# dorukb/Advanced-CPU-Raytracing

Measured on AMD Instinct MI355X. Metric: Mrays/sec + achieved HBM GB/s fraction, 1920×1080 primary+shadow rays, higher is better.
Workload: dtype f32; 1 GPU; synthetic height field K=100352 tris, 1920x1080, 1 spp, 1 point light, default Blinn-Phong, primary+shadow rays; scene_K=100352, width=1920, height=1080, spp=1, rays_per_frame=4147193, camera_rays=2073600, frames_in_flight=16

## Files before the change

advanced-cpu-raytracing_amd/csrc/rtg_common.hpp:

```cpp
#pragma once
#include <hip/hip_runtime.h>
#include <stdint.h>

#include "rtg_device.hpp"

#ifndef RTG_MEGA_WAVES
#define RTG_MEGA_WAVES 2
#endif
#if RTG_MEGA_WAVES > 2 && !defined(RTG_MEGA_WAVES_EXPERIMENTAL)
#error "RTG_MEGA_WAVES > 2 is experimental (round-1 scratch fault, DESIGN.md §7): add -DRTG_MEGA_WAVES_EXPERIMENTAL=1"
#endif
#ifndef RTG_LEAN_WAVES
#define RTG_LEAN_WAVES 8
#endif
#ifndef RTG_SHADE_WAVES
#define RTG_SHADE_WAVES 3
#endif
#ifndef RTG_TREE_SHADE_WAVES
#define RTG_TREE_SHADE_WAVES 1
#endif
#ifndef RTG_BIGLEAF_LEAN
#define RTG_BIGLEAF_LEAN 0
#endif
#ifndef RTG_INST_WAVES
// ... 344 lines not shown
        hit = tt & (t > 0.0f) & (t < limit);
    }
    const bool unsure = !no & !tt;
    if (__builtin_expect(__ballot(unsure) != 0, 0)) {
        if (unsure) hit = tri_test_rec(R, r, limit, tout);
    }
    return hit;
}

DEV float tri_test_pk(const float4* R, const Ray& r, float limit, float& tout, float onf) {
    const float4 A = R[0], E1 = R[1], E2 = R[2];
    const float dx = r.d.x, dy = r.d.y, dz = r.d.z;
    const float detA = det3(E1.x, E2.x, dx, E1.y, E2.y, dy, E1.z, E2.z, dz);
    const float ad = fabsf(detA);
    const float rd = __builtin_amdgcn_rcpf(detA);
    const float sx = A.x - r.o.x, sy = A.y - r.o.y, sz = A.z - r.o.z;
    const float nb = det3(sx, E2.x, dx, sy, E2.y, dy, sz, E2.z, dz);
    const float ng = det3(E1.x, sx, dx, E1.y, sy, dy, E1.z, sz, dz);
    const float beta = nb * rd, gama = ng * rd, sum = gama + beta;
    const float sslack = fmaf(0x1p-19f, sum, 0x1p-22f);
    const float rng = __builtin_elementwise_minimum(ad - 0x1p-100f, 0x1p100f - ad);
    const float ttv = __builtin_elementwise_minimum(vmin3(beta - 1e-30f, gama - 1e-30f, (1.0f - sum) - sslack),
                                                    __builtin_elementwise_minimum(rng, onf));
    const float rjv = __builtin_elementwise_minimum(fmaxf(fmaxf(-1e-30f - beta, -1e-30f - gama), (sum - 1.0f) - sslack),
                                                    rng);
    float hv = -1.0f;
    if (__ballot(ttv > 0.0f)) {
        const float t = det3(E1.x, E2.x, sx, E1.y, E2.y, sy, E1.z, E2.z, sz) / detA;
        tout = t;
        hv = vmin3(ttv, t, limit - t);
    }
    const bool unsure = (onf > 0.0f) & !(ttv > 0.0f) & !(rjv > 0.0f) & (detA != 0.0f);
    if (__builtin_expect(__ballot(unsure) != 0, 0)) {
        if (unsure) hv = tri_test_rec(R, r, limit, tout) ? 1.0f : -1.0f;
    }
    return hv;
}

typedef int rtg_s16 __attribute__((ext_vector_type(16)));
typedef int rtg_s8 __attribute__((ext_vector_type(8)));
typedef int rtg_s4 __attribute__((ext_vector_type(4)));
DEV const void* uniform_ptr(const void* p) {
    const uint64_t v = (uint64_t)p;
    const uint32_t lo = __builtin_amdgcn_readfirstlane((uint32_t)v), hi = __builtin_amdgcn_readfirstlane((uint32_t)(v >> 32));
    return (const void*)(((uint64_t)hi << 32) | lo);
}
DEV void sload_wnode(const WNode* p, rtg_s16& a, rtg_s16& b) {
    asm volatile("s_load_dwordx16 %0, %2, 0x0\n\ts_load_dwordx16 %1, %2, 0x40\n\ts_waitcnt lgkmcnt(0)"
                 : "=&s"(a), "=&s"(b) : "s"(uniform_ptr(p)) : "memory");
}
DEV void sload_rec(const float4* p, rtg_s8& a, rtg_s4& b) {
    asm volatile("s_load_dwordx8 %0, %2, 0x0\n\ts_load_dwordx4 %1, %2, 0x20\n\ts_waitcnt lgkmcnt(0)"
                 : "=&s"(a), "=&s"(b) : "s"(uniform_ptr(p)) : "memory");
}
DEV void sload_node(const float4* p, rtg_s8& a) {
    asm volatile("s_load_dwordx8 %0, %1, 0x0\n\ts_waitcnt lgkmcnt(0)" : "=&s"(a) : "s"(uniform_ptr(p)) : "memory");
}
DEV float4 f4(int x, int y, int z, int w) {
    return make_float4(__int_as_float(x), __int_as_float(y), __int_as_float(z), __int_as_float(w));
}
DEV uint64_t hit_key(float t, int f) { return ((uint64_t)__float_as_uint(t) << 32) | (uint32_t)f; }

DEV uint64_t shfl64(uint64_t v, int src) {
    const uint32_t lo = (uint32_t)__shfl((int)(uint32_t)v, src);
    const uint32_t hi = (uint32_t)__shfl((int)(uint32_t)(v >> 32), src);
    return ((uint64_t)hi << 32) | lo;
}
DEV uint64_t wave_min_key(uint64_t key, uint64_t em) {
    if (em == ~0ull) {
        const int lane = threadIdx.x & 63;
        for (int m = 1; m < 64; m <<= 1) {
            const uint64_t other = shfl64(key, lane ^ m);
            if (other < key) key = other;
        }
        return key;
    }
    uint64_t acc = ~0ull;
    while (em) {
        const int l = __ffsll((long long)em) - 1;
        em &= em - 1;
        const uint64_t v = shfl64(key, l);
        if (v < acc) acc = v;
    }
    return acc;
}

#ifndef RTG_SEQ_SEL
#define RTG_SEQ_SEL 1
#endif
template <bool ANY, bool STATS, bool SEL = RTG_SEQ_SEL != 0>
DEV bool walk_bvh_seq(const DevScene& S, int i, const int end, const Ray& r, float& minT, int& hitFace, float limit,
                      Cnt<STATS>& c) {
    bool hit = false;
    const RayRcp q = ray_rcp(r);
    while (i < end) {
        const float4 a = S.nodes[2 * i];
        const float4 b = S.nodes[2 * i + 1];
        c.template node<ANY>();
        const int skip = __float_as_int(b.z);
        if (box_hit_fast<SEL>(a.x, a.y, a.z, a.w, b.x, b.y, r, q, minT)) {
            const int leaf = __float_as_int(b.w);
            if (leaf >= 0) {
                int first = leaf >> 8, cnt = leaf & 255;
                if (leaf == LEAF_EXT) {
                    const int2 e = S.node_ext[i];
                    first = e.x;
                    cnt = e.y;
                }
                for (int f = first; f < first + cnt; ++f) {
                    c.template tri<ANY>();
                    float t;
                    if (SEL ? tri_test_sel(S.tris + 3 * f, r, minT, t) : tri_test_fast(S, f, r, minT, t)) {
                        minT = t;
                        hitFace = f;
                        hit = true;
                        if (ANY && t < limit) return true;
                    }
                }
                i = skip;
            } else {
                i = i + 1;
            }
        } else {
            i = skip;
        }
    }
    return hit;
}


struct SlabRay {
    f3 o;
    float ix, iy, iz;
};
DEV SlabRay slab_ray(const Ray& r, const RayRcp& q) {
    SlabRay s;
    s.o = r.o;
    s.ix = q.ix; s.iy = q.iy; s.iz = q.iz;
    return s;
}
DEV bool slab_cons(float lx, float ly, float lz, float hx, float hy, float hz, const SlabRay& s, float minTc,
                   float& tnear) {
    const float tx1 = (lx - s.o.x) * s.ix, tx2 = (hx - s.o.x) * s.ix;
    const float ty1 = (ly - s.o.y) * s.iy, ty2 = (hy - s.o.y) * s.iy;
    const float tz1 = (lz - s.o.z) * s.iz, tz2 = (hz - s.o.z) * s.iz;
    const float tmin = fmaxf(fmaxf(fminf(tx1, tx2), fminf(ty1, ty2)), fminf(tz1, tz2));
    const float tmax = fminf(fminf(fmaxf(tx1, tx2), fmaxf(ty1, ty2)), fmaxf(tz1, tz2));
    tnear = tmin;
    return (tmax > -1e-30f) & (tmax >= fmaf(tmin, 1.0f - 0x1p-21f, -1e-30f)) & (tmin < minTc);
}

struct CoopEvent {
    float ox, oy, oz, dx, dy, dz, minT;
    int first, cnt, start;
    unsigned long long best;
};
DEV void wave_lds_sync() {
    __builtin_amdgcn_fence(__ATOMIC_RELEASE, "wavefront");
    __builtin_amdgcn_wave_barrier();
    __builtin_amdgcn_fence(__ATOMIC_ACQUIRE, "wavefront");
}
DEV uint64_t coop_leaf_tests(const DevScene& S, uint64_t coop, const Ray& r, float minT, int first, int cnt) {
    __shared__ CoopEvent table[4][64];
    CoopEvent* E = table[threadIdx.x >> 6];
    const uint64_t em = __ballot(1);
    const int lane = threadIdx.x & 63;
    const int nact = __popcll(em);
    const int rank = __popcll(em & ((1ull << lane) - 1ull));
    const int ne = __popcll(coop);
    const int slot = cnt > 0 ? __popcll(coop & ((1ull << lane) - 1ull)) : -1;
    if (slot >= 0) {
        CoopEvent& e = E[slot];
        e.ox = r.o.x; e.oy = r.o.y; e.oz = r.o.z;
        e.dx = r.d.x; e.dy = r.d.y; e.dz = r.d.z;
        e.minT = minT;
        e.first = first;
        e.cnt = cnt;
        e.best = ~0ull;
    }
    wave_lds_sync();
    int total = 0, start = 0;
    for (int k = 0; k < ne; ++k) {
        if (k == slot) start = total;
        total += E[k].cnt;
    }
    if (slot >= 0) E[slot].start = start;
    wave_lds_sync();
    for (int w = rank; w < total; w += nact) {
        int lo = 0, hi = ne - 1;
        while (lo < hi) {
            const int mid = (lo + hi + 1) >> 1;
            if (E[mid].start <= w) lo = mid;
            else hi = mid - 1;
        }
        const CoopEvent& e = E[lo];
        Ray lr;
        lr.o = mk(e.ox, e.oy, e.oz);
        lr.d = mk(e.dx, e.dy, e.dz);
        const int f = e.first + (w - e.start);
        float t;
        if (tri_test_fast(S, f, lr, e.minT, t)) atomicMin(&E[lo].best, (unsigned long long)hit_key(t, f));
    }
    wave_lds_sync();
    const uint64_t mine = slot >= 0 ? (uint64_t)E[slot].best : ~0ull;
    wave_lds_sync();
    return mine;
}

template <bool ANY, bool STATS, bool COOP>
DEV bool walk_bvh(const DevScene& S, int i, const int end, const Ray& r, float& minT, int& hitFace, float limit,
                  Cnt<STATS>& c) {
    if constexpr (!COOP) return walk_bvh_seq<ANY, STATS>(S, i, end, r, minT, hitFace, limit, c);
    if (!S.coop) return walk_bvh_seq<ANY, STATS, false>(S, i, end, r, minT, hitFace, limit, c);
    bool hit = false;
    const RayRcp q = ray_rcp(r);
    bool active = i < end;
    while (__ballot(active)) {
        int coopFirst = 0, coopCnt = 0;
        if (active) {
            const float4 a = S.nodes[2 * i];
            const float4 b = S.nodes[2 * i + 1];
            c.template node<ANY>();
            const int skip = __float_as_int(b.z);
            if (box_hit_fast(a.x, a.y, a.z, a.w, b.x, b.y, r, q, minT)) {
                const int leaf = __float_as_int(b.w);
                if (leaf >= 0) {
                    int first = leaf >> 8, cnt = leaf & 255;
                    if (leaf == LEAF_EXT) {
                        const int2 e = S.node_ext[i];
                        first = e.x;
                        cnt = e.y;
                    }
                    if (cnt > kCoopLeaf) {
                        coopFirst = first;
                        coopCnt = cnt;
                    } else {
                        for (int f = first; f < first + cnt; ++f) {
                            c.template tri<ANY>();
                            float t;
                            if (tri_test_fast(S, f, r, minT, t)) {
                                minT = t;
                                hitFace = f;
                                hit = true;
                                if (ANY && t < limit) {
                                    active = false;
                                    break;
                                }
                            }
                        }
                    }
                    i = skip;
                } else {
                    i = i + 1;
                }
            } else {
                i = skip;
            }
            if (i >= end) active = false;
        }
        const uint64_t coop = __ballot(coopCnt > 0);
        if (coop) {
            const uint64_t best = coop_leaf_tests(S, coop, r, minT, coopFirst, coopCnt);
            if (coopCnt > 0) {
                c.template tri_n<ANY>((uint32_t)coopCnt);
                if (best != ~0ull) {
                    minT = __uint_as_float((uint32_t)(best >> 32));
                    hitFace = (int)(uint32_t)best;
                    hit = true;
                    if (ANY && minT < limit) active = false;
                }
            }
        }
    }
    return hit;
}

DEV int wave_min_int(int v) {
    for (int m = 1; m < 64; m <<= 1) {
        const int o = __shfl_xor(v, m);
        v = o < v ? o : v;
    }
    return v;
}

constexpr int kDeferLeaf = 16;
template <int BYTES, typename T>
DEV const T* rec_at(const T* base, int i) {
    return (const T*)((const char*)base + (uint32_t)i * (uint32_t)BYTES);
}
#ifndef RTG_DEFER_LANES
#define RTG_DEFER_LANES 16
#endif
struct DeferCtx {
    float4* e;
    int* count;
    int cap;
    int ray;
    bool deferred;
};
DEV uint64_t obj_key(float t, int k, int f) {
    return ((uint64_t)__float_as_uint(t) << 32) | ((uint64_t)(uint32_t)k << 20) | (uint64_t)((uint32_t)f & 0xFFFFFu);
}

template <bool ANY, bool STATS, bool SC = false, bool DEFER = false>
DEV bool walk_bvh_packet(const DevScene& S, int begin, int end, const Ray& r, float& minT, int& hitFace,
                         float limit, Cnt<STATS>& c, DeferCtx* dc = nullptr, int k = 0) {
    begin = __builtin_amdgcn_readfirstlane(begin);
    end = __builtin_amdgcn_readfirstlane(end);
    const int face0 = hitFace;
    bool hit = false;
    const RayRcp q = ray_rcp(r);
    const SlabFma sf = slab_fma(r, q);
    const float slack0 = slab_slack0(sf, q.fast);
    const int kDone = 0x7FFFFFFF;
    int resume = begin;
    int i = begin;
    while (i < end) {
        bool act = resume <= i;
        if (ANY && !__ballot(act)) {
            const int all = __ballot(1) == ~0ull ? wave_min_int(resume) : [&] {
                int m = kDone;
                uint64_t em = __ballot(1);
                while (em) {
                    const int l = __ffsll((long long)em) - 1;
                    em &= em - 1;
                    const int v = __shfl(resume, l);
                    m = v < m ? v : m;
                }
                return m;
            }();
            i = __builtin_amdgcn_readfirstlane(all);
            continue;
        }
        i = __builtin_amdgcn_readfirstlane(i);
        const int ip1 = i + 1;
        float4 a, b;
        int ndr[8];
        if constexpr (SC) {
            rtg_s8 nd;
            sload_node(rec_at<32>(S.nodes, i), nd);
            a = f4(nd[0], nd[1], nd[2], nd[3]);
            b = f4(nd[4], nd[5], nd[6], nd[7]);
#pragma unroll
            for (int u = 0; u < 8; ++u) ndr[u] = nd[u];
        } else {
            a = S.nodes[2 * i];
            b = S.nodes[2 * i + 1];
        }
        const int skip = __float_as_int(b.z);
        const int leaf = __float_as_int(b.w);
        bool pass;
        if constexpr (SC) {
            if (act) c.template node<ANY>();
            pass = box_pass_pk(a.x, a.y, a.z, a.w, b.x, b.y, r, sf, minT, ip1 - resume, slack0);
            resume = max(resume, pass ? 0 : skip);
        } else {
            pass = false;
            if (act) {
                c.template node<ANY>();
                pass = box_hit_fast(a.x, a.y, a.z, a.w, b.x, b.y, r, q, minT);
                if (!pass) resume = skip;
            }
        }
        const int cur = i;
        int lf;
        {
            const uint64_t pm = __builtin_amdgcn_ballot_w64(pass);
            int nx;
            asm("s_cmp_lg_u64 %[pm], 0\n\t"
                "s_cselect_b32 %[lf], %[leaf], 0\n\t"
                "s_cmp_lt_i32 %[lf], 0\n\t"
                "s_cselect_b32 %[nx], %[ip1], %[skip]"
                : [lf] "=&s"(lf), [nx] "=&s"(nx)
                : [pm] "s"(pm), [leaf] "s"(leaf), [ip1] "s"(ip1), [skip] "s"(skip)
                : "scc");
            i = nx;
        }
        if (lf > 0) {
            {
                int first = leaf >> 8, cnt = leaf & 255;
                if (leaf == LEAF_EXT) {
                    const int2 e = S.node_ext[cur];
                    first = __builtin_amdgcn_readfirstlane(e.x);
                    cnt = __builtin_amdgcn_readfirstlane(e.y);
                }
                if constexpr (DEFER) {
                    const uint64_t m = __ballot(pass);
                    if (cnt > kDeferLeaf && __popcll(m) <= RTG_DEFER_LANES) {
                        const int lane = threadIdx.x & 63, lead = __ffsll((long long)m) - 1;
                        int base = 0;
                        if (lane == lead) base = atomicAdd(dc->count, __popcll(m));
                        base = __shfl(base, lead);
                        const int slot = base + __popcll(m & ((1ull << lane) - 1ull));
                        if (pass && slot < dc->cap) {
                            float4* q = dc->e + 3 * (size_t)slot;
                            q[0] = make_float4(r.o.x, r.o.y, r.o.z, minT);
                            q[1] = make_float4(r.d.x, r.d.y, r.d.z, __int_as_float(dc->ray));
                            q[2] = make_float4(__int_as_float(first), __int_as_float(cnt), __int_as_float(k), 0.f);
                            dc->deferred = true;
                            pass = false;
                        }
                    }
                }
                for (int f = first; f < first + cnt; ++f) {
                    if constexpr (SC) {
                        rtg_s8 ra;
                        rtg_s4 rb;
                        sload_rec(rec_at<48>(S.tris, f), ra, rb);
                        const float4 R[3] = {f4(ra[0], ra[1], ra[2], ra[3]), f4(ra[4], ra[5], ra[6], ra[7]),
                                             f4(rb[0], rb[1], rb[2], rb[3])};
                        if (pass) c.template tri<ANY>();
                        float t;
                        const bool ok = tri_test_pk(R, r, minT, t, pass ? 1.0f : -1.0f) > 0.0f;
                        minT = ok ? t : minT;
                        hitFace = ok ? f : hitFace;
                        if (ANY) {
                            const bool fin = ok & (t < limit);
                            pass &= !fin;
                            resume = fin ? kDone : resume;
                        }
                    } else if (pass) {
                        c.template tri<ANY>();
                        float t;
                        if (tri_test_fast(S, f, r, minT, t)) {
                            minT = t;
                            hitFace = f;
                            hit = true;
                            if (ANY && t < limit) {
                                pass = false;
                                resume = kDone;
                            }
                        }
                    }
                }
            }
        }
    }
    if constexpr (SC) return hit | (hitFace != face0);
    return hit;
}

#ifndef RTG_XFORM_LAUNDER
#define RTG_XFORM_LAUNDER 1
#endif
DEV bool sphere_t(const DevObject& ob, const Ray& lr, float minT, float& tout) {
    const f3 center = mk(ob.center[0], ob.center[1], ob.center[2]);
    const float radius = ob.center[3];
    f3 oc = sub(lr.o, center);
    float c = dot(oc, oc) - (radius * radius);
    float b = 2 * dot(lr.d, oc);
    float a = dot(lr.d, lr.d);
    float delta = b * b - (4 * a * c);
    if (delta < 0.0f) return false;
    delta = sqrtf(delta);
    a = (float)(2.0 * a);
    float t1 = (-b + delta) / a;
    float t2 = (-b - delta) / a;
    float t = t1 < t2 ? t1 : t2;
    if (t1 < t2) { t = (t1 > 0.0f) ? t1 : t2; }
    else if (t2 < t1) { t = (t2 > 0.0f) ? t2 : t1; }
    tout = t;
    return t < minT && t > 0.0f;
}

template <bool MOTION = true>
DEV Ray local_ray(const DevObject& ob, const Ray& r, float mbTime) {
    Ray lr;
    lr.o = xform(ob.inv, r.o, 1.0f);
    lr.d = xform(ob.inv, r.d, 0.0f);
    if (MOTION && (ob.flags & OBJF_MOTION_BLUR)) lr.o = add(lr.o, muls(ld3(ob.mbv), mbTime));
    return lr;
}
DEV Ray trav_ray(const DevObject& ob, const Ray& r0, float mbTime) {
    Ray r = r0;
#if RTG_XFORM_LAUNDER
    asm volatile("" : "+v"(r.o.x), "+v"(r.o.y), "+v"(r.o.z), "+v"(r.d.x), "+v"(r.d.y), "+v"(r.d.z));
#endif
    if (!(ob.flags & OBJF_IDENTITY)) return local_ray(ob, r, mbTime);
    Ray lr = ident_ray(r);
    if (ob.flags & OBJF_MOTION_BLUR) lr.o = add(lr.o, muls(ld3(ob.mbv), mbTime));
    return lr;
}

struct Hit {
    float t;
    int obj, face;
    f3 o;
};

template <bool ANY, bool STATS, int FEAT = FEAT_ALL, bool PK = false, bool DEFER = false>
DEV bool trace(const DevScene& S, Ray& r, float mbTime, float minT, float limit, Hit& h, Cnt<STATS>& c,
               DeferCtx* dc = nullptr) {
    h.t = minT;
    h.obj = -1;
    h.face = -1;
    const RayRcp rq = (FEAT & FEAT_INSTANCE) ? ray_rcp(r) : RayRcp{};
    int gskip = 0;
    for (int k = 0; k < S.num_objects; ++k) {
        const DevObject& ob = S.objects[k];
        if ((FEAT & FEAT_INSTANCE) && ob.group_end > k) {
            const float4 ga = S.group_box[2 * k], gb = S.group_box[2 * k + 1];
            if constexpr (PK) {
                if (k >= gskip && !box_hit_fast(ga.x, ga.y, ga.z, gb.x, gb.y, gb.z, r, rq, h.t)) gskip = ob.group_end;
                if (!__ballot(k >= gskip)) {
                    k = ob.group_end - 1;
                    continue;
                }
            } else if (!box_hit_fast(ga.x, ga.y, ga.z, gb.x, gb.y, gb.z, r, rq, h.t)) {
                k = ob.group_end - 1;
                continue;
            }
        }
        if (PK && k < gskip) continue;
        c.obj();
        if ((FEAT & FEAT_SPHERE) && ob.kind == OBJ_SPHERE) {
            c.sph();
            Ray lr = trav_ray(ob, r, mbTime);
            float t;
            if (sphere_t(ob, lr, h.t, t)) {
                h.t = t; h.obj = k; h.face = -1; h.o = r.o;
                if (ANY && t < limit) return true;
            }
            continue;
        }
        if (ANY && (ob.flags & OBJF_SHADOW_SKIP)) continue;
        if ((FEAT & FEAT_INSTANCE) && ob.kind == OBJ_INSTANCE) {
            Ray wr = r;
            if (ob.flags & OBJF_MOTION_BLUR) wr.o = add(wr.o, muls(ld3(ob.mbv), mbTime));
            if (!box_hit_fast(ob.bmin[0], ob.bmin[1], ob.bmin[2], ob.bmax[0], ob.bmax[1], ob.bmax[2], wr, rq, h.t)) {
                r.o = wr.o;
                continue;
            }
        }
        Ray lr = (FEAT & FEAT_XFORM) ? trav_ray(ob, r, mbTime) : ident_ray(r);
        int face = -1;
        float t = h.t;
        bool found;
        if constexpr (PK)
            found = walk_bvh_packet<ANY, STATS, RTG_PRIMARY_PACKET == 2, DEFER>(S, ob.node_begin, ob.node_end, lr, t,
                                                                                  face, limit, c, dc, k);
        else found = walk_bvh<ANY, STATS, (FEAT & FEAT_BIGLEAF) != 0>(S, ob.node_begin, ob.node_end, lr, t, face, limit, c);
        if (found) {
            h.t = t; h.obj = k; h.face = face; h.o = r.o;
            if (ANY && t < limit) return true;
        }
    }
    return !ANY && h.obj >= 0;
}

#ifndef RTG_WIDE_WAVES_PLAIN
#define RTG_WIDE_WAVES_PLAIN 7
#endif
#ifndef RTG_INST_ANY_WAVES
#define RTG_INST_ANY_WAVES 6
#endif
#define RTG_WIDE_WAVES(FEAT) (((FEAT) & FEAT_INSTANCE) ? RTG_INST_ANY_WAVES : RTG_WIDE_WAVES_PLAIN)


#ifndef RTG_DEFER_ANY_LANES
#define RTG_DEFER_ANY_LANES 16
#endif
#ifndef RTG_DEFER_ANY_LEAF
#define RTG_DEFER_ANY_LEAF 16
#endif
struct AnyDefer {
    float4* e;
    int* count;
    int cap;
    int q;
    bool deferred;
};
#define RTG_PK_STACK 64
#ifndef RTG_PK_MAX_STEPS
#define RTG_PK_MAX_STEPS 4096
#endif
struct SlabCons {
    float ix, iy, iz;
    float ax, ay, az, bx, by, bz;
    bool ok;
};
DEV SlabCons slab_cons_ray(const Ray& r, const RayRcp& q) {
    SlabCons s;
    const float px = r.o.x * q.ix, py = r.o.y * q.iy, pz = r.o.z * q.iz;
    const float ex = copysignf(0x1p-22f * fabsf(px), q.ix), ey = copysignf(0x1p-22f * fabsf(py), q.iy),
                ez = copysignf(0x1p-22f * fabsf(pz), q.iz);
    s.ix = q.ix; s.iy = q.iy; s.iz = q.iz;
    s.ax = -px - ex; s.ay = -py - ey; s.az = -pz - ez;
    s.bx = -px + ex; s.by = -py + ey; s.bz = -pz + ez;
    s.ok = fmaxf(fmaxf(fabsf(px), fabsf(py)), fabsf(pz)) <= 0x1p100f;
    return s;
}
DEV float slab_cons_v(float lx, float ly, float lz, float hx, float hy, float hz, const SlabCons& s, float minTc,
                      float& tnear, float livef) {
    const float tx1 = fmaf(lx, s.ix, s.ax), tx2 = fmaf(hx, s.ix, s.bx);
    const float ty1 = fmaf(ly, s.iy, s.ay), ty2 = fmaf(hy, s.iy, s.by);
    const float tz1 = fmaf(lz, s.iz, s.az), tz2 = fmaf(hz, s.iz, s.bz);
    const float tmin = fmaxf(fmaxf(fminf(tx1, tx2), fminf(ty1, ty2)), fminf(tz1, tz2));
    const float tmax = fminf(fminf(fmaxf(tx1, tx2), fmaxf(ty1, ty2)), fmaxf(tz1, tz2));
    tnear = tmin;
    return __builtin_elementwise_minimum(
        vmin3(tmax + 1e-30f, (tmax - fmaf(tmin, 1.0f - 0x1p-20f, -1e-30f)) + 1e-30f, minTc - tmin), livef);
}

template <bool STATS, bool DEFER = false>
DEV int walk_wide_any_pk(const DevScene& S, int node, const Ray& lr, float minT0, float limit, bool inst_conf,
                         Cnt<STATS>& c, AnyDefer* ad = nullptr) {
    const RayRcp q = ray_rcp(lr);
    const SlabCons sr = slab_cons_ray(lr, q);
    const bool fast = q.fast & sr.ok;
    const float minTc = minT0 * (1.0f + 0x1p-20f);
    const float icf = inst_conf ? 1.0f : -1.0f;
    float livef = fast ? 1.0f : -1.0f;
    int und = fast ? 0 : 1;
    __shared__ int pk_stack[4][RTG_PK_STACK];
    int* const stk = pk_stack[(threadIdx.x >> 6) & 3];
    int sp = 0;
    node = __builtin_amdgcn_readfirstlane(node);
    int steps = 0;
    while (__ballot(livef > 0.0f)) {
        if (++steps > RTG_PK_MAX_STEPS) {
            und |= livef > 0.0f;
            break;
        }
        node = __builtin_amdgcn_readfirstlane(node);
        rtg_s16 na, nb;
        sload_wnode(rec_at<128>(S.anodes, node), na, nb);
        if (livef > 0.0f) c.wnode();
        float tn[4], hv[4];
#pragma unroll
        for (int k = 0; k < 4; ++k)
            hv[k] = slab_cons_v(__int_as_float(na[k]), __int_as_float(na[8 + k]), __int_as_float(nb[k]),
                                __int_as_float(na[4 + k]), __int_as_float(na[12 + k]), __int_as_float(nb[4 + k]), sr,
                                minTc, tn[k], livef);
        const int lead = __ffsll((long long)__ballot(livef > 0.0f)) - 1;
        int next = -1;
        float nextT = INFINITY;
#pragma unroll
        for (int k = 0; k < 4; ++k) {
            const int cr = nb[8 + k], lfw = nb[12 + k];
            float hk = hv[k];
            if (cr == WCHILD_EMPTY || !__ballot(hk > 0.0f)) continue;
            if (cr >= 0) {
                const float t = __int_as_float(__builtin_amdgcn_readlane(__float_as_int(tn[k]), lead));
                int spill = cr;
                if (t < nextT) {
                    spill = next;
                    next = cr;
                    nextT = t;
                }
                if (spill >= 0) {
                    if (sp < RTG_PK_STACK) {
                        if ((int)(threadIdx.x & 63) == lead) stk[sp] = spill;
                        ++sp;
                    } else {
                        und |= livef > 0.0f;
                    }
                }
                continue;
            }
            const int first = lfw >> 8, cnt = lfw & 255;
            if constexpr (DEFER) {
                const uint64_t m = __ballot(hk > 0.0f);
                if (cnt > RTG_DEFER_ANY_LEAF && __popcll(m) <= RTG_DEFER_ANY_LANES) {
                    const int lane = threadIdx.x & 63, ld = __ffsll((long long)m) - 1;
                    int base = 0;
                    if (lane == ld) base = atomicAdd(ad->count, __popcll(m));
                    base = __shfl(base, ld);
                    const int slot = base + __popcll(m & ((1ull << lane) - 1ull));
                    if (hk > 0.0f && slot < ad->cap) {
                        float4* qe = ad->e + 3 * (size_t)slot;
                        qe[0] = make_float4(lr.o.x, lr.o.y, lr.o.z, minT0);
                        qe[1] = make_float4(lr.d.x, lr.d.y, lr.d.z, limit);
                        qe[2] = make_float4(__int_as_float(first), __int_as_float(cnt), __int_as_float(ad->q),
                                            __int_as_float((int)inst_conf));
                        ad->deferred = true;
                        hk = -1.0f;
                    }
                }
            }
            for (int e = first; e < first + cnt; ++e) {
                rtg_s8 ra;
                rtg_s4 rb;
                sload_rec(rec_at<48>(S.ahtris, e), ra, rb);
                if (hk > 0.0f) c.template tri<true>();
                const float4 R[3] = {f4(ra[0], ra[1], ra[2], ra[3]), f4(ra[4], ra[5], ra[6], ra[7]), f4(rb[0], rb[1], rb[2], rb[3])};
                float t;
                const float okv = tri_test_pk(R, lr, limit, t, hk);
                if (!__ballot(okv > 0.0f)) continue;
                rtg_s8 rn;
                sload_node(rec_at<32>(S.nodes, ra[3]), rn);
                Ray er = lr;
                asm volatile("" : "+v"(er.o.x), "+v"(er.o.y), "+v"(er.o.z));
                const SlabFma sf = slab_fma(er, q);
                const float slack0 = slab_slack0(sf, true);
                const float rv = box_pass_v(__int_as_float(rn[0]), __int_as_float(rn[1]), __int_as_float(rn[2]),
                                            __int_as_float(rn[3]), __int_as_float(rn[4]), __int_as_float(rn[5]), er, sf,
                                            minT0, okv, slack0);
                const float sv = box_pass_v(__int_as_float(rn[0]), __int_as_float(rn[1]), __int_as_float(rn[2]),
                                            __int_as_float(rn[3]), __int_as_float(rn[4]), __int_as_float(rn[5]), er, sf,
                                            limit, __builtin_elementwise_minimum(rv, icf), slack0);
                const bool suff = sv > 0.0f;
                livef = suff ? -2.0f : livef;
                hk = suff ? -1.0f : hk;
                und |= (rv > 0.0f) & !suff;
            }
        }
        if (!__ballot(livef > 0.0f)) break;
        if (next >= 0) {
            node = next;
            continue;
        }
        if (sp == 0) break;
        node = stk[--sp];
    }
    return livef < -1.5f ? 1 : (und ? -1 : 0);
}

template <bool STATS, int FEAT, bool DEFER = false>
DEV int trace_any_wide(const DevScene& S, const Ray& r, float minT0, float limit, Cnt<STATS>& c,
                       AnyDefer* ad = nullptr) {
    const RayRcp rq = (FEAT & FEAT_INSTANCE) ? ray_rcp(r) : RayRcp{};
    if ((FEAT & FEAT_INSTANCE) && !rq.fast) return -1;
    bool undecided = false;
    int gskip = 0;
    for (int k = 0; k < S.num_objects; ++k) {
        const DevObject& ob = S.objects[k];
        if ((FEAT & FEAT_INSTANCE) && ob.group_end > k) {
            const float4 ga = S.group_box[2 * k], gb = S.group_box[2 * k + 1];
            if (k >= gskip && !box_hit_fast(ga.x, ga.y, ga.z, gb.x, gb.y, gb.z, r, rq, minT0))
                gskip = ob.group_end;
            if (!__ballot(k >= gskip)) {
                k = ob.group_end - 1;
                continue;
            }
        }
        if (k < gskip) continue;
        c.obj();
        if ((FEAT & FEAT_SPHERE) && ob.kind == OBJ_SPHERE) {
            c.sph();
            Ray lr = trav_ray(ob, r, 0.f);
            float t;
            if (sphere_t(ob, lr, limit, t)) return 1;
            continue;
        }
        if (ob.flags & OBJF_SHADOW_SKIP) continue;
        bool conf = true;
        if ((FEAT & FEAT_INSTANCE) && ob.kind == OBJ_INSTANCE) {
            if (!box_hit_fast(ob.bmin[0], ob.bmin[1], ob.bmin[2], ob.bmax[0], ob.bmax[1], ob.bmax[2], r, rq, minT0))
                continue;
            conf = box_hit_fast(ob.bmin[0], ob.bmin[1], ob.bmin[2], ob.bmax[0], ob.bmax[1], ob.bmax[2], r, rq, limit);
        }
        const Ray lr = (FEAT & FEAT_XFORM) ? trav_ray(ob, r, 0.f) : ident_ray(r);
        if (ob.aroot < 0) return -1;
        const int res = walk_wide_any_pk<STATS, DEFER>(S, ob.aroot, lr, minT0, limit, conf, c, ad);
        if (res > 0) return 1;
        undecided |= res < 0;
    }
    return undecided ? -1 : 0;
}

DEV float next_up(float x) { return x == INFINITY ? x : __uint_as_float(__float_as_uint(x) + 1u); }

DEV bool hit_less(float t, int k, int f, float bt, int bk, int bf) {
    return (t < bt) | ((t == bt) & ((k < bk) | ((k == bk) & (f < bf))));
}
DEV bool slab_cons2(float lx, float ly, float lz, float hx, float hy, float hz, const SlabRay& s, float minTc,
                    float& tnear, bool& hinf) {
    const float tx1 = (lx - s.o.x) * s.ix, tx2 = (hx - s.o.x) * s.ix;
    const float ty1 = (ly - s.o.y) * s.iy, ty2 = (hy - s.o.y) * s.iy;
    const float tz1 = (lz - s.o.z) * s.iz, tz2 = (hz - s.o.z) * s.iz;
    const float tmin = fmaxf(fmaxf(fminf(tx1, tx2), fminf(ty1, ty2)), fminf(tz1, tz2));
    const float tmax = fminf(fminf(fmaxf(tx1, tx2), fmaxf(ty1, ty2)), fmaxf(tz1, tz2));
    tnear = tmin;
    hinf = (tmax > -1e-30f) & (tmax >= fmaf(tmin, 1.0f - 0x1p-21f, -1e-30f));
    return hinf & (tmin < minTc);
}
DEV float wave_min_pos(float v) {
    uint32_t u = __float_as_uint(v);
    for (int m = 1; m < 64; m <<= 1) {
        const uint32_t o = (uint32_t)__shfl_xor((int)u, m);
        u = o < u ? o : u;
    }
    return __uint_as_float(u);
}
DEV float cull_limit(float t) { return t * (1.0f + 0x1p-20f); }

struct ClosestState {
    float bestT, hidT, cullMin;
    int bestK, bestF, hidK, hidF;
};

template <bool STATS>
DEV bool walk_closest_pk(const DevScene& S, int node, const int k, const Ray& lr, const RayRcp& q, const SlabRay& sr,
                         ClosestState& B, Cnt<STATS>& c) {
    __shared__ int ck_node[4][RTG_PK_STACK];
    __shared__ float ck_tn[4][RTG_PK_STACK];
    int* const stk = ck_node[(threadIdx.x >> 6) & 3];
    float* const stn = ck_tn[(threadIdx.x >> 6) & 3];
    const bool writer = (int)(threadIdx.x & 63) == __ffsll((long long)__ballot(1)) - 1;
    int sp = 0;
    int steps = 0;
    node = __builtin_amdgcn_readfirstlane(node);
    while (true) {
        if (++steps > RTG_PK_MAX_STEPS) return false;
        node = __builtin_amdgcn_readfirstlane(node);
        rtg_s16 na, nb;
        sload_wnode(rec_at<128>(S.anodes, node), na, nb);
        const float4 lox = f4(na[0], na[1], na[2], na[3]), hix = f4(na[4], na[5], na[6], na[7]);
        const float4 loy = f4(na[8], na[9], na[10], na[11]), hiy = f4(na[12], na[13], na[14], na[15]);
        const float4 loz = f4(nb[0], nb[1], nb[2], nb[3]), hiz = f4(nb[4], nb[5], nb[6], nb[7]);
        const int cidx[4] = {nb[8], nb[9], nb[10], nb[11]};
        const int lidx[4] = {nb[12], nb[13], nb[14], nb[15]};
        c.ewnode();
        const float minTc = cull_limit(B.bestT);
        float tn[4];
        bool h[4], hi[4];
        h[0] = slab_cons2(lox.x, loy.x, loz.x, hix.x, hiy.x, hiz.x, sr, minTc, tn[0], hi[0]);
        h[1] = slab_cons2(lox.y, loy.y, loz.y, hix.y, hiy.y, hiz.y, sr, minTc, tn[1], hi[1]);
        h[2] = slab_cons2(lox.z, loy.z, loz.z, hix.z, hiy.z, hiz.z, sr, minTc, tn[2], hi[2]);
        h[3] = slab_cons2(lox.w, loy.w, loz.w, hix.w, hiy.w, hiz.w, sr, minTc, tn[3], hi[3]);
#pragma unroll
        for (int j = 0; j < 4; ++j) {
            if (cidx[j] == WCHILD_EMPTY || cidx[j] >= 0) continue;
            if (hi[j] & !h[j]) B.cullMin = fminf(B.cullMin, tn[j]);
            if (!__ballot(h[j])) continue;
            const int first = lidx[j] >> 8, cnt = lidx[j] & 255;
            for (int e = first; e < first + cnt; ++e) {
                rtg_s8 ra;
                rtg_s4 rb;
                sload_rec(rec_at<48>(S.ahtris, e), ra, rb);
                const float4 R[3] = {f4(ra[0], ra[1], ra[2], ra[3]), f4(ra[4], ra[5], ra[6], ra[7]),
                                     f4(rb[0], rb[1], rb[2], rb[3])};
                const int f = ra[7];
                if (h[j]) c.template tri<false>();
                float t;
                const bool ok = h[j] & tri_test_sel(R, lr, INFINITY, t, h[j]);
                const bool better = ok && hit_less(t, k, f, B.bestT, B.bestK, B.bestF);
                if (!__ballot(better)) continue;
                rtg_s8 rn;
                sload_node(rec_at<32>(S.nodes, ra[3]), rn);
                const float bx0 = __int_as_float(rn[0]), by0 = __int_as_float(rn[1]), bz0 = __int_as_float(rn[2]);
                const float bx1 = __int_as_float(rn[3]), by1 = __int_as_float(rn[4]), bz1 = __int_as_float(rn[5]);
                const bool vis = better & box_hit_fast<true>(bx0, by0, bz0, bx1, by1, bz1, lr, q, next_up(t), better);
                const bool hcand = better & !vis;
                const bool hid = hcand & box_hit_fast<true>(bx0, by0, bz0, bx1, by1, bz1, lr, q, INFINITY, hcand);
                if (vis) { B.bestT = t; B.bestK = k; B.bestF = f; }
                if (hid && hit_less(t, k, f, B.hidT, B.hidK, B.hidF)) { B.hidT = t; B.hidK = k; B.hidF = f; }
            }
        }
        const float minTc2 = cull_limit(B.bestT);
        bool h2[4];
#pragma unroll
        for (int j = 0; j < 4; ++j) {
            const bool inner = cidx[j] >= 0;
            h2[j] = inner & h[j] & (tn[j] < minTc2);
            if (inner & hi[j] & !h2[j]) B.cullMin = fminf(B.cullMin, tn[j]);
        }
        const uint64_t any = __ballot(h2[0] | h2[1] | h2[2] | h2[3]);
        int next = -1;
        if (any) {
            const int lead = __ffsll((long long)any) - 1;
            float nextT = INFINITY, nextTw = INFINITY;
#pragma unroll
            for (int j = 0; j < 4; ++j) {
                if (!__ballot(h2[j])) continue;
                const float tl = __int_as_float(__builtin_amdgcn_readlane(__float_as_int(h2[j] ? tn[j] : INFINITY), lead));
                const float tw = wave_min_pos(h2[j] ? fmaxf(tn[j], 0.0f) : INFINITY);
                int spill = cidx[j];
                float spillT = tw;
                if (next < 0 || tl < nextT) {
                    spill = next;
                    spillT = nextTw;
                    next = cidx[j];
                    nextT = tl;
                    nextTw = tw;
                }
                if (spill >= 0) {
                    if (sp >= RTG_PK_STACK) return false;
                    if (writer) { stk[sp] = spill; stn[sp] = spillT; }
                    ++sp;
                }
            }
        }
        if (next >= 0) {
            node = next;
            continue;
        }
        bool found = false;
        while (sp > 0) {
            --sp;
            const int n = stk[sp];
            const float tw = stn[sp];
            if (__ballot(tw < cull_limit(B.bestT))) {
                node = n;
                found = true;
                break;
            }
            B.cullMin = fminf(B.cullMin, tw);
        }
        if (!found) break;
    }
    return true;
}

// ... 869 lines not shown
```

Before: 17820 Mrays/s.

## Add lean packet BVH walker for closest-hit on plain triangle scenes

Adds a specialized closest-hit packet traversal used when the scene has no spheres, instances or transforms and the SC variant is selected. Interior nodes use a conservative FMA slab test, falling back to the exact box test only on NaN lanes. The next-node choice is computed with scalar inline assembly, and the resume/any-hit bookkeeping is dropped. The aim is fewer VALU instructions and branches per node visit, at the cost of relying on the conservative test's precision and on hand-written scalar asm.

```diff
diff --git a/advanced-cpu-raytracing_amd/csrc/rtg_common.hpp b/advanced-cpu-raytracing_amd/csrc/rtg_common.hpp
--- a/advanced-cpu-raytracing_amd/csrc/rtg_common.hpp
+++ b/advanced-cpu-raytracing_amd/csrc/rtg_common.hpp
@@ -670,9 +670,14 @@
     return ((uint64_t)__float_as_uint(t) << 32) | ((uint64_t)(uint32_t)k << 20) | (uint64_t)((uint32_t)f & 0xFFFFFu);
 }
 
-template <bool ANY, bool STATS, bool SC = false, bool DEFER = false>
+template <bool DEFER>
+DEV bool walk_bvh_packet_lx(const DevScene& S, int begin, int end, const Ray& r, float& minT, int& hitFace,
+                            DeferCtx* dc, int k);
+
+template <bool ANY, bool STATS, bool SC = false, bool DEFER = false, bool LX = false>
 DEV bool walk_bvh_packet(const DevScene& S, int begin, int end, const Ray& r, float& minT, int& hitFace,
                          float limit, Cnt<STATS>& c, DeferCtx* dc = nullptr, int k = 0) {
+    if constexpr (LX && SC && !ANY && !STATS) return walk_bvh_packet_lx<DEFER>(S, begin, end, r, minT, hitFace, dc, k);
     begin = __builtin_amdgcn_readfirstlane(begin);
     end = __builtin_amdgcn_readfirstlane(end);
     const int face0 = hitFace;
@@ -904,9 +909,10 @@
         int face = -1;
         float t = h.t;
         bool found;
+        constexpr bool LX = !(FEAT & (FEAT_SPHERE | FEAT_INSTANCE | FEAT_XFORM));
         if constexpr (PK)
-            found = walk_bvh_packet<ANY, STATS, RTG_PRIMARY_PACKET == 2, DEFER>(S, ob.node_begin, ob.node_end, lr, t,
-                                                                                  face, limit, c, dc, k);
+            found = walk_bvh_packet<ANY, STATS, RTG_PRIMARY_PACKET == 2, DEFER, LX>(S, ob.node_begin, ob.node_end, lr,
+                                                                                      t, face, limit, c, dc, k);
         else found = walk_bvh<ANY, STATS, (FEAT & FEAT_BIGLEAF) != 0>(S, ob.node_begin, ob.node_end, lr, t, face, limit, c);
         if (found) {
             h.t = t; h.obj = k; h.face = face; h.o = r.o;
@@ -968,6 +974,100 @@
     tnear = tmin;
     return __builtin_elementwise_minimum(
         vmin3(tmax + 1e-30f, (tmax - fmaf(tmin, 1.0f - 0x1p-20f, -1e-30f)) + 1e-30f, minTc - tmin), livef);
+}
+
+DEV float slab_cons_pk(float lx, float ly, float lz, float hx, float hy, float hz, const SlabCons& s, float minTc) {
+    const float tx1 = fmaf(lx, s.ix, s.ax), tx2 = fmaf(hx, s.ix, s.bx);
+    const float ty1 = fmaf(ly, s.iy, s.ay), ty2 = fmaf(hy, s.iy, s.by);
+    const float tz1 = fmaf(lz, s.iz, s.az), tz2 = fmaf(hz, s.iz, s.bz);
+    const float tmin = fmaxf(fmaxf(fminf(tx1, tx2), fminf(ty1, ty2)), fminf(tz1, tz2));
+    const float tmax = fminf(fminf(fmaxf(tx1, tx2), fmaxf(ty1, ty2)), fmaxf(tz1, tz2));
+    return vmin3(tmax + 1e-30f, (tmax - fmaf(tmin, 1.0f - 0x1p-20f, -1e-30f)) + 1e-30f, minTc - tmin);
+}
+template <bool DEFER>
+DEV bool walk_bvh_packet_lx(const DevScene& S, int begin, int end, const Ray& r, float& minT, int& hitFace,
+                            DeferCtx* dc, int k) {
+    begin = __builtin_amdgcn_readfirstlane(begin);
+    end = __builtin_amdgcn_readfirstlane(end);
+    const int face0 = hitFace;
+    const RayRcp q = ray_rcp(r);
+    const SlabCons sc = slab_cons_ray(r, q);
+    const SlabFma sf = slab_fma(r, q);
+    const float slack0 = slab_slack0(sf, q.fast);
+    const float kc = (q.fast & sc.ok) ? 1.0f + 0x1p-20f : __builtin_nanf("");
+    float minTc = minT * kc;
+    int i = begin;
+    while (i < end) {
+        i = __builtin_amdgcn_readfirstlane(i);
+        const int ip1 = i + 1;
+        rtg_s8 nd;
+        sload_node(rec_at<32>(S.nodes, i), nd);
+        const float4 a = f4(nd[0], nd[1], nd[2], nd[3]), b = f4(nd[4], nd[5], nd[6], nd[7]);
+        const int skip = nd[6], leaf = nd[7];
+        float pv;
+        if (leaf < 0) {
+            pv = slab_cons_pk(a.x, a.y, a.z, a.w, b.x, b.y, sc, minTc);
+            if (__builtin_expect(__ballot(pv != pv) != 0, 0)) {
+                if (pv != pv) pv = box_hit(a.x, a.y, a.z, a.w, b.x, b.y, r, minT) ? 1.0f : -1.0f;
+            }
+        } else {
+            pv = box_pass_v(a.x, a.y, a.z, a.w, b.x, b.y, r, sf, minT, INFINITY, slack0);
+        }
+        bool pass = pv > 0.0f;
+        const int cur = i;
+        int lf;
+        {
+            const uint64_t pm = __builtin_amdgcn_ballot_w64(pass);
+            int nx;
+            asm("s_cmp_lg_u64 %[pm], 0\n\t"
+                "s_cselect_b32 %[lf], %[leaf], 0\n\t"
+                "s_cmp_lt_i32 %[lf], 0\n\t"
+                "s_cselect_b32 %[nx], %[ip1], %[skip]"
+                : [lf] "=&s"(lf), [nx] "=&s"(nx)
+                : [pm] "s"(pm), [leaf] "s"(leaf), [ip1] "s"(ip1), [skip] "s"(skip)
+                : "scc");
+            i = nx;
+        }
+        if (lf > 0) {
+            int first = leaf >> 8, cnt = leaf & 255;
+            if (leaf == LEAF_EXT) {
+                const int2 e = S.node_ext[cur];
+                first = __builtin_amdgcn_readfirstlane(e.x);
+                cnt = __builtin_amdgcn_readfirstlane(e.y);
+            }
+            if constexpr (DEFER) {
+                const uint64_t m = __ballot(pass);
+                if (cnt > kDeferLeaf && __popcll(m) <= RTG_DEFER_LANES) {
+                    const int lane = threadIdx.x & 63, lead = __ffsll((long long)m) - 1;
+                    int base = 0;
+                    if (lane == lead) base = atomicAdd(dc->count, __popcll(m));
+                    base = __shfl(base, lead);
+                    const int slot = base + __popcll(m & ((1ull << lane) - 1ull));
+                    if (pass && slot < dc->cap) {
+                        float4* qe = dc->e + 3 * (size_t)slot;
+                        qe[0] = make_float4(r.o.x, r.o.y, r.o.z, minT);
+                        qe[1] = make_float4(r.d.x, r.d.y, r.d.z, __int_as_float(dc->ray));
+                        qe[2] = make_float4(__int_as_float(first), __int_as_float(cnt), __int_as_float(k), 0.f);
+                        dc->deferred = true;
+                        pass = false;
+                    }
+                }
+            }
+            for (int f = first; f < first + cnt; ++f) {
+                rtg_s8 ra;
+                rtg_s4 rb;
+                sload_rec(rec_at<48>(S.tris, f), ra, rb);
+                const float4 R[3] = {f4(ra[0], ra[1], ra[2], ra[3]), f4(ra[4], ra[5], ra[6], ra[7]),
+                                     f4(rb[0], rb[1], rb[2], rb[3])};
+                float t;
+                const bool ok = tri_test_pk(R, r, minT, t, pass ? 1.0f : -1.0f) > 0.0f;
+                minT = ok ? t : minT;
+                hitFace = ok ? f : hitFace;
+            }
+            minTc = minT * kc;
+        }
+    }
+    return hitFace != face0;
 }
 
 template <bool STATS, bool DEFER = false>
```

New measurement: 18990 Mrays/s, median of 6. 1.07x the previous value.
